# modin-project/modin

Measured on NVIDIA H100. Metric: rows/sec elementwise map (a*b+c) on 5e8x8 f64, higher is better.
Workload: dtype f64

## Files before the change

### modin_b200/csrc/elementwise.cu

```cuda
#include <type_traits>

#include "common.cuh"

namespace mb200 {

constexpr int kThreads = 256;
constexpr int kPair = 2;
constexpr int kSlab = kThreads * kPair;
constexpr int kSlabs = 8;
constexpr int kTile = kSlab * kSlabs;

struct MapParams {
  const void* in0[MB200_MAX_COLS];
  const void* in1[MB200_MAX_COLS];
  const void* in2[MB200_MAX_COLS];
  void* out[MB200_MAX_COLS];
  uint64_t s0[MB200_MAX_COLS];
  uint64_t s1[MB200_MAX_COLS];
  long long nrows;
};

template <typename T>
__device__ __forceinline__ T from_bits(uint64_t b);
template <>
__device__ __forceinline__ double from_bits<double>(uint64_t b) {
  return __longlong_as_double((long long)b);
}
template <>
__device__ __forceinline__ long long from_bits<long long>(uint64_t b) {
  return (long long)b;
}
template <>
__device__ __forceinline__ uint8_t from_bits<uint8_t>(uint64_t b) {
  return (uint8_t)(b != 0);
}

constexpr __host__ __device__ int op_nin(int op) { return op >= 64 ? 3 : (op >= 32 ? 2 : 1); }
constexpr __host__ __device__ bool op_is_pred(int op) {
  return op == MB200_OP_ISNA || op == MB200_OP_NOTNA || (op >= MB200_OP_EQ_S && op <= MB200_OP_GE_S) ||
         (op >= MB200_OP_EQ && op <= MB200_OP_GE);
}

template <int OP, typename TI, typename TO>
__device__ __forceinline__ TO apply(TI a, TI b, TI c, TI s0, TI s1) {
  constexpr bool F = std::is_same<TI, double>::value;
  if constexpr (OP == MB200_OP_ABS) {
    if constexpr (F) return (TO)fabs(a);
    else return (TO)(a < 0 ? (TI)(0ULL - (unsigned long long)a) : a);
  } else if constexpr (OP == MB200_OP_NEG) {
    if constexpr (F) return (TO)__longlong_as_double(__double_as_longlong(a) ^ (long long)0x8000000000000000ULL);
    else return (TO)(TI)(0ULL - (unsigned long long)a);
  } else if constexpr (OP == MB200_OP_ISNA) {
    return (TO)(a != a);
  } else if constexpr (OP == MB200_OP_NOTNA) {
    return (TO)(a == a);
  } else if constexpr (OP == MB200_OP_FILLNA_S) {
    return (TO)((a != a) ? s0 : a);
  } else if constexpr (OP == MB200_OP_AFFINE) {
    if constexpr (F) return (TO)__dadd_rn(__dmul_rn(a, s0), s1);
    else return (TO)(TI)((unsigned long long)a * (unsigned long long)s0 + (unsigned long long)s1);
  } else if constexpr (OP == MB200_OP_ADD_S || OP == MB200_OP_ADD) {
    TI r = (OP == MB200_OP_ADD) ? b : s0;
    if constexpr (F) return (TO)__dadd_rn(a, r);
    else return (TO)(TI)((unsigned long long)a + (unsigned long long)r);
  } else if constexpr (OP == MB200_OP_SUB_S || OP == MB200_OP_SUB) {
    TI r = (OP == MB200_OP_SUB) ? b : s0;
    if constexpr (F) return (TO)__dsub_rn(a, r);
    else return (TO)(TI)((unsigned long long)a - (unsigned long long)r);
  } else if constexpr (OP == MB200_OP_RSUB_S) {
    if constexpr (F) return (TO)__dsub_rn(s0, a);
    else return (TO)(TI)((unsigned long long)s0 - (unsigned long long)a);
  } else if constexpr (OP == MB200_OP_MUL_S || OP == MB200_OP_MUL) {
    TI r = (OP == MB200_OP_MUL) ? b : s0;
// ... 49 lines not shown
    return (TO)((a != a) ? b : a);
  } else if constexpr (OP == MB200_OP_FMA3) {
    if constexpr (F) return (TO)__dadd_rn(__dmul_rn(a, b), c);
    else return (TO)(TI)((unsigned long long)a * (unsigned long long)b + (unsigned long long)c);
  } else {
    return (TO)a;
  }
}

template <typename T>
struct Pair;
template <>
struct Pair<double> {
  using type = double2;
  static __device__ __forceinline__ double2 load(const double* p) { return ldg_stream_f64x2(p); }
  static __device__ __forceinline__ void store(double* p, const double2& v) { stg_stream_f64x2(p, v); }
};
template <>
struct Pair<long long> {
  using type = longlong2;
  static __device__ __forceinline__ longlong2 load(const long long* p) { return ldg_stream_i64x2(p); }
  static __device__ __forceinline__ void store(long long* p, const longlong2& v) { stg_stream_i64x2(p, v); }
};
template <>
struct Pair<uint8_t> {
  using type = uchar2;
  static __device__ __forceinline__ uchar2 load(const uint8_t* p) { return __ldg(reinterpret_cast<const uchar2*>(p)); }
  static __device__ __forceinline__ void store(uint8_t* p, const uchar2& v) { *reinterpret_cast<uchar2*>(p) = v; }
};

template <int OP, typename TI, typename TO, bool VEC>
__global__ void __launch_bounds__(kThreads) map_kernel(const __grid_constant__ MapParams p) {
  constexpr int NIN = op_nin(OP);
  const int tid = threadIdx.x;
  const int col = blockIdx.y;
  const long long base = (long long)blockIdx.x * kTile;
  const TI* __restrict__ a = static_cast<const TI*>(p.in0[col]);
  const TI* __restrict__ b = NIN >= 2 ? static_cast<const TI*>(p.in1[col]) : nullptr;
  const TI* __restrict__ c = NIN >= 3 ? static_cast<const TI*>(p.in2[col]) : nullptr;
  TO* __restrict__ o = static_cast<TO*>(p.out[col]);
  const TI s0 = from_bits<TI>(p.s0[col]);
  const TI s1 = from_bits<TI>(p.s1[col]);
  if (VEC && base + kTile <= p.nrows) {
    typename Pair<TI>::type va[kSlabs], vb[kSlabs], vc[kSlabs];
#pragma unroll
    for (int k = 0; k < kSlabs; ++k) {
      const long long i = base + k * kSlab + kPair * tid;
      va[k] = Pair<TI>::load(a + i);
      if constexpr (NIN >= 2) vb[k] = Pair<TI>::load(b + i);
      if constexpr (NIN >= 3) vc[k] = Pair<TI>::load(c + i);
    }
#pragma unroll
    for (int k = 0; k < kSlabs; ++k) {
      const long long i = base + k * kSlab + kPair * tid;
      TI bx = 0, by = 0, cx = 0, cy = 0;
      if constexpr (NIN >= 2) bx = vb[k].x, by = vb[k].y;
      if constexpr (NIN >= 3) cx = vc[k].x, cy = vc[k].y;
      typename Pair<TO>::type r;
      r.x = apply<OP, TI, TO>(va[k].x, bx, cx, s0, s1);
      r.y = apply<OP, TI, TO>(va[k].y, by, cy, s0, s1);
      Pair<TO>::store(o + i, r);
    }
  } else {
    const long long end = (base + kTile < p.nrows) ? base + kTile : p.nrows;
    for (long long i = base + tid; i < end; i += kThreads) {
      TI x = a[i];
      TI y = NIN >= 2 ? b[i] : (TI)0;
      TI z = NIN >= 3 ? c[i] : (TI)0;
      o[i] = apply<OP, TI, TO>(x, y, z, s0, s1);
    }
  }
}

#define MB_CASE(OPC, TI, TO)                                     \
  case OPC:                                                      \
    if (vec)                                                     \
      map_kernel<OPC, TI, TO, true><<<grid, kThreads, 0, st>>>(p);  \
    else                                                         \
      map_kernel<OPC, TI, TO, false><<<grid, kThreads, 0, st>>>(p); \
    MB_LAUNCH_CHECK("map_kernel");                               \
    return 0;

}

using namespace mb200;

extern "C" int mb200_map(int op, int dtype, int ncols, const void* const* in0, const void* const* in1,
                         const void* const* in2, void* const* out, int64_t nrows, const uint64_t* s0,
                         const uint64_t* s1, mb200_stream_t stream) {
  if (ncols < 0 || ncols > MB200_MAX_COLS) return fail("mb200_map", "ncols out of range (0..32)");
  if (nrows < 0) return fail("mb200_map", "negative nrows");
  if (ncols == 0 || nrows == 0) return 0;
  if (!in0 || !out) return fail("mb200_map", "null column array");
  const int nin = op_nin(op);
  if (nin >= 2 && !in1) return fail("mb200_map", "binary op needs in1");
  if (nin >= 3 && !in2) return fail("mb200_map", "ternary op needs in2");
  MapParams p;
  memset(&p, 0, sizeof(p));
  bool vec = true;
  for (int c = 0; c < ncols; ++c) {
    p.in0[c] = in0[c];
    p.in1[c] = nin >= 2 ? in1[c] : nullptr;
    p.in2[c] = nin >= 3 ? in2[c] : nullptr;
    p.out[c] = out[c];
    p.s0[c] = s0 ? s0[c] : 0;
    p.s1[c] = s1 ? s1[c] : 0;
    if (!in0[c] || !out[c]) return fail("mb200_map", "null column pointer");
    vec = vec && aligned16(in0[c]) && aligned16(out[c]);
    if (nin >= 2) vec = vec && in1[c] && aligned16(in1[c]);
    if (nin >= 3) vec = vec && in2[c] && aligned16(in2[c]);
    if ((nin >= 2 && !in1[c]) || (nin >= 3 && !in2[c])) return fail("mb200_map", "null column pointer");
  }
  p.nrows = nrows;
  const long long tiles_per_col = (nrows + kTile - 1) / kTile;
  if (tiles_per_col > 0x7fffffffLL) return fail("mb200_map", "too many rows for one launch");
  const dim3 grid((unsigned)tiles_per_col, (unsigned)ncols);
  cudaStream_t st = (cudaStream_t)stream;

  if (dtype == MB200_F64) {
    switch (op) {
      MB_CASE(MB200_OP_ABS, double, double)
      MB_CASE(MB200_OP_NEG, double, double)
      MB_CASE(MB200_OP_ISNA, double, uint8_t)
      MB_CASE(MB200_OP_NOTNA, double, uint8_t)
      MB_CASE(MB200_OP_FILLNA_S, double, double)
      MB_CASE(MB200_OP_AFFINE, double, double)
      MB_CASE(MB200_OP_ADD_S, double, double)
      MB_CASE(MB200_OP_SUB_S, double, double)
      MB_CASE(MB200_OP_RSUB_S, double, double)
      MB_CASE(MB200_OP_MUL_S, double, double)
      MB_CASE(MB200_OP_DIV_S, double, double)
      MB_CASE(MB200_OP_RDIV_S, double, double)
      MB_CASE(MB200_OP_EQ_S, double, uint8_t)
      MB_CASE(MB200_OP_NE_S, double, uint8_t)
      MB_CASE(MB200_OP_LT_S, double, uint8_t)
      MB_CASE(MB200_OP_LE_S, double, uint8_t)
      MB_CASE(MB200_OP_GT_S, double, uint8_t)
      MB_CASE(MB200_OP_GE_S, double, uint8_t)
      MB_CASE(MB200_OP_CLIP_S, double, double)
      MB_CASE(MB200_OP_COPY, double, double)
      MB_CASE(MB200_OP_ROUND_S, double, double)
      MB_CASE(MB200_OP_ORDERED_S, double, long long)
      MB_CASE(MB200_OP_ADD, double, double)
      MB_CASE(MB200_OP_SUB, double, double)
      MB_CASE(MB200_OP_MUL, double, double)
      MB_CASE(MB200_OP_DIV, double, double)
      MB_CASE(MB200_OP_EQ, double, uint8_t)
      MB_CASE(MB200_OP_NE, double, uint8_t)
      MB_CASE(MB200_OP_LT, double, uint8_t)
// ... 57 lines not shown
```

### modin_b200/csrc/groupby.cu

```cuda
#include "common.cuh"

namespace mb200 {

int sort_pairs_device(long long* keys, long long* pay, long long* tmp_keys, long long* tmp_pay,
                      unsigned int* counts, long long n, unsigned long long bias, int nbits, cudaStream_t st);
size_t sort_scratch_bytes(long long n);

struct __align__(16) Slot {
  long long key;
  int gid;
  int pad;
};

struct GbMeta {
  int ngroups;
  int overflow;
  long long kmin;
  long long kmax;
};

}

struct mb200_gb_table {
  mb200::Slot* slots;
  long long cap;
  double* acc;
  long long* cnt;
  long long* size;
  long long gcap;
  int nvals;
  int vstride;
  int flags;
  mb200::GbMeta* meta;
  int dense;
  long long kbase;
  unsigned int* present;
  long long nwords;
  unsigned int* blockoff;
  int borrowed;
  int skewed;
  int persisted;
  size_t carve_bytes, window_bytes;
  long long win_lo, win_hi;
  void* arena;
  size_t arena_bytes;
};

namespace mb200 {

constexpr int kGbThreads = 256;
constexpr int kGbWarps = kGbThreads / 32;
constexpr int kColStride = 34;
constexpr int kTileRows = 256;
constexpr int kTileColStride = 258;
constexpr int kGbStages = 3;
constexpr int kGbTmaThreads = kGbThreads + 32;
constexpr int kStageBytes = ((9 * kTileColStride * 8 + 127) / 128) * 128;

struct GbParams {
  Slot* slots;
  unsigned int mask;
  long long cap;
  double* acc;
  long long* cnt;
  long long* size;
  long long gcap;
  int nvals;
  int vstride;
  int flags;
  GbMeta* meta;
  const long long* keys;
  const void* vals[MB200_MAX_COLS];
  const void* pcnt[MB200_MAX_COLS];
  const long long* psize;
  long long nrows;
  int dense;
  long long kbase;
  unsigned int* present;
  int policy_mode;
  int prefetch;
};

__device__ __forceinline__ void red_add_f64(double* p, double v, uint64_t pol) {
  if (pol)
    asm volatile("red.relaxed.gpu.global.add.L2::cache_hint.f64 [%0], %1, %2;" ::"l"(p), "d"(v), "l"(pol) : "memory");
  else
    asm volatile("red.relaxed.gpu.global.add.f64 [%0], %1;" ::"l"(p), "d"(v) : "memory");
}
__device__ __forceinline__ void red_add_u64(long long* p, long long v, uint64_t) {
  asm volatile("red.relaxed.gpu.global.add.u64 [%0], %1;" ::"l"(p), "l"(v) : "memory");
// ... 234 lines not shown
            if (p.flags & MB200_GB_COUNT) {
              if (PARTIAL) red_add_u64(p.cnt + o, static_cast<const long long*>(p.pcnt[c0 + c])[base + r], keep);
              else if (xv == xv) red_add_u64(p.cnt + o, 1LL, keep);
            }
          }
        }
        if (p.dense && !(p.flags & MB200_GB_SIZE)) {
          seen |= __shfl_xor_sync(0xffffffffu, seen, 1);
          seen |= __shfl_xor_sync(0xffffffffu, seen, 2);
          seen |= __shfl_xor_sync(0xffffffffu, seen, 4);
          const unsigned int unseen = ~seen & rowok;
          if (c == 0 && unseen) {
#pragma unroll
            for (int kk = 0; kk < 8; ++kk)
              if ((unseen >> kk) & 1u) dense_mark(p, gs[kk]);
          }
        }
        __syncwarp();
      }
    }
  }
}

constexpr int kHotSlots = 256;
constexpr int kHotStride = 9;
constexpr int kHotStages = 2;
__host__ __device__ constexpr int hot_offset(int stages) {
  return ((stages * kStageBytes + 2 * stages * 8 + 63) / 64) * 64;
}
constexpr int kHotBytesSum = kHotSlots * 4 + kHotSlots * kHotStride * 8;
constexpr int kHotBytes = kHotBytesSum + kHotSlots * kHotStride * 4;
constexpr int kHotBit = 1 << 30;

template <bool HOT, int STAGES>
__global__ void __launch_bounds__(kGbTmaThreads) gb_accumulate_tma_kernel(const __grid_constant__ GbParams p,
                                                                          long long ntiles) {
  extern __shared__ __align__(128) unsigned char smem_raw[];
  uint64_t* full = reinterpret_cast<uint64_t*>(smem_raw + STAGES * kStageBytes);
  uint64_t* empty = full + STAGES;
  int* s_tag = reinterpret_cast<int*>(smem_raw + hot_offset(STAGES));
  double* s_hot = reinterpret_cast<double*>(smem_raw + hot_offset(STAGES) + kHotSlots * 4);
  unsigned int* s_hcnt = reinterpret_cast<unsigned int*>(smem_raw + hot_offset(STAGES) + kHotSlots * 4 + kHotSlots * kHotStride * 8);
  const int tid = threadIdx.x, lane = tid & 31, warp = tid >> 5;
  const int nv = p.nvals;
  const int gcap = (int)p.gcap;
  const long long first = blockIdx.x;
  const long long nmine = first < ntiles ? (ntiles - first + gridDim.x - 1) / gridDim.x : 0;

  if (HOT) {
    for (int i = tid; i < kHotSlots; i += kGbTmaThreads) s_tag[i] = -1;
    for (int i = tid; i < kHotSlots * kHotStride; i += kGbTmaThreads) {
      s_hot[i] = 0.0;
      if (p.flags & MB200_GB_COUNT) s_hcnt[i] = 0u;
    }
  }
  if (tid == 0) {
#pragma unroll
    for (int s = 0; s < STAGES; ++s) {
      mbar_init(&full[s], 1);
      mbar_init(&empty[s], kGbWarps);
    }
    mbar_fence_init();
  }
  __syncthreads();

  if (warp == kGbWarps) {
    if (lane == 0) {
      const uint64_t pol = l2_policy_evict_first();
      for (long long k = 0; k < nmine; ++k) {
        const int s = (int)(k % STAGES);
        if (k >= STAGES) mbar_wait(&empty[s], (uint32_t)(((k / STAGES) - 1) & 1));
        const long long row0 = (first + k * gridDim.x) * kTileRows;
        double* stage = reinterpret_cast<double*>(smem_raw + (size_t)s * kStageBytes);
        mbar_expect_tx(&full[s], (uint32_t)((1 + nv) * kTileRows * 8));
        tma_bulk_g2s(stage, p.keys + row0, kTileRows * 8, &full[s], pol);
        for (int c = 0; c < nv; ++c)
          tma_bulk_g2s(stage + (size_t)(1 + c) * kTileColStride, static_cast<const double*>(p.vals[c]) + row0,
                       kTileRows * 8, &full[s], pol);
      }
    }
    return;
  }
  const uint64_t keep = table_policy(p.policy_mode);
  const int c = lane & 7;
  for (long long k = 0; k < nmine; ++k) {
    const int s = (int)(k % STAGES);
    mbar_wait(&full[s], (uint32_t)((k / STAGES) & 1));
    const double* stage = reinterpret_cast<const double*>(smem_raw + (size_t)s * kStageBytes);
    const long long key = reinterpret_cast<const long long*>(stage)[warp * 32 + lane];
    if (p.prefetch && k + 1 < nmine) {
      const int s1 = (int)((k + 1) % STAGES);
      mbar_wait(&full[s1], (uint32_t)(((k + 1) / STAGES) & 1));
      const long long nk =
          reinterpret_cast<const long long*>(smem_raw + (size_t)s1 * kStageBytes)[warp * 32 + lane];
      const Slot* ns = &p.slots[hash_key(nk) & p.mask];
      asm volatile("prefetch.global.L2 [%0];" ::"l"(ns));
    }
    int gid = resolve_gid(p, key, keep);
    if ((p.flags & MB200_GB_SIZE) && gid < gcap) red_add_u64(p.size + gid, 1LL, keep);
    if (HOT && gid < gcap) {
      const int slot = gid & (kHotSlots - 1);
      int tag = *reinterpret_cast<volatile int*>(&s_tag[slot]);
      if (tag == -1) {
        const int old = atomicCAS(&s_tag[slot], -1, gid);
        tag = old == -1 ? gid : old;
      }
      if (tag == gid) gid |= kHotBit;
    }
    const double* vt = stage + kTileColStride + warp * 32;
    unsigned int seen = 0;
    int gs[8];
#pragma unroll
    for (int kk = 0; kk < 8; ++kk) {
      const int r = 4 * kk + (lane >> 3);
      const int pg = __shfl_sync(0xffffffffu, gid, r);
      const int g = HOT ? (pg & ~kHotBit) : pg;
      gs[kk] = g;
      if (c < nv && g < gcap) {
        const double xv = vt[c * kTileColStride + r];
        if (dense_visible(p, xv)) seen |= 1u << kk;
        if (xv == xv) {
          if (HOT && (pg & kHotBit)) {
            const int o = (g & (kHotSlots - 1)) * kHotStride + c;
            if (p.flags & MB200_GB_SUM) atomicAdd(&s_hot[o], xv);
            if (p.flags & MB200_GB_COUNT) atomicAdd(&s_hcnt[o], 1u);
          } else {
            const size_t o = (size_t)g * p.vstride + c;
            acc_update(p, o, xv, keep);
            if (p.flags & MB200_GB_COUNT) red_add_u64(p.cnt + o, 1LL, keep);
          }
        }
      }
    }
    if (p.dense && !(p.flags & MB200_GB_SIZE)) {
      seen |= __shfl_xor_sync(0xffffffffu, seen, 1);
      seen |= __shfl_xor_sync(0xffffffffu, seen, 2);
      seen |= __shfl_xor_sync(0xffffffffu, seen, 4);
      unsigned int unseen = ~seen & 0xffu;
      if (c == 0 && unseen) {
#pragma unroll
        for (int kk = 0; kk < 8; ++kk)
          if (((unseen >> kk) & 1u) && gs[kk] < gcap) dense_mark(p, gs[kk]);
      }
    }
    __syncwarp();
    if (lane == 0) mbar_arrive(&empty[s]);
  }
  if (HOT) {
    asm volatile("bar.sync 1, %0;" ::"n"(kGbThreads) : "memory");
    for (int i = tid; i < kHotSlots * 8; i += kGbThreads) {
      const int slot = i >> 3, cc = i & 7;
      const int tag = s_tag[slot];
      if (tag < 0 || cc >= nv) continue;
      const size_t o = (size_t)tag * p.vstride + cc;
      if (p.flags & MB200_GB_SUM) red_add_f64(p.acc + o, s_hot[slot * kHotStride + cc], 0);
      if ((p.flags & MB200_GB_COUNT) && s_hcnt[slot * kHotStride + cc])
        red_add_u64(p.cnt + o, (long long)s_hcnt[slot * kHotStride + cc], 0);
    }
  }
}

constexpr int kSmemThreads = 1024;

struct SmemTableLayout {
  unsigned int acc_off, cnt_off, size_off, present_off, total;
  int svs;
  int nrep;
  int rstride;
  int zstride;
};

__global__ void __launch_bounds__(kSmemThreads, 1) gb_accumulate_smem_kernel(const __grid_constant__ GbParams p,
                                                                             const SmemTableLayout lay) {
  extern __shared__ __align__(16) unsigned char smem_raw[];
// ... 68 lines not shown
      for (int r = 1; r < nrep; ++r) a += s_acc[r * rstride + o];
      red_add_f64(p.acc + i, a, 0);
    } else if (f_min || f_max) {
      long long a = s_acc_i[o];
      for (int r = 1; r < nrep; ++r) {
        const long long b = s_acc_i[r * rstride + o];
        a = f_min ? (b < a ? b : a) : (b > a ? b : a);
      }
      if (f_min && a != 0x7fffffffffffffffLL) red_min_s64(reinterpret_cast<long long*>(p.acc) + i, a);
      if (f_max && a != (long long)0x8000000000000000ULL) red_max_s64(reinterpret_cast<long long*>(p.acc) + i, a);
    }
    if (f_cnt) {
      long long n = 0;
      for (int r = 0; r < nrep; ++r) n += s_cnt[r * rstride + o];
      if (n) red_add_u64(p.cnt + i, n, 0);
    }
  }
  for (int g = tid; g < R; g += kSmemThreads) {
    if (!s_present[g]) continue;
    reinterpret_cast<unsigned char*>(p.present)[g] = 1;
    if (f_size) {
      long long n = 0;
      for (int r = 0; r < nrep; ++r) n += s_size[r * zstride + g];
      red_add_u64(p.size + g, n, 0);
    }
  }
}

__global__ void gb_fill_kernel(long long* p, long long n, long long v) {
  const long long stride = (long long)gridDim.x * blockDim.x;
  for (long long i = (long long)blockIdx.x * blockDim.x + threadIdx.x; i < n; i += stride) p[i] = v;
}

__global__ void gb_init_kernel(Slot* slots, long long cap, GbMeta* meta) {
  const long long i = (long long)blockIdx.x * blockDim.x + threadIdx.x;
  if (i < cap) {
    Slot s;
    s.key = 0;
    s.gid = -1;
    s.pad = 0;
    slots[i] = s;
  }
  if (i == 0) {
    meta->ngroups = 0;
    meta->overflow = 0;
    meta->kmin = 0x7fffffffffffffffLL;
    meta->kmax = (long long)0x8000000000000000ULL;
  }
}

__global__ void __launch_bounds__(256) gb_collect_kernel(const Slot* __restrict__ slots, long long cap, long long gcap,
                                                         long long* __restrict__ keys_by_gid,
                                                         long long* __restrict__ perm, GbMeta* meta) {
  __shared__ long long s_min[8], s_max[8];
  const long long i = (long long)blockIdx.x * blockDim.x + threadIdx.x;
  long long lo = 0x7fffffffffffffffLL, hi = (long long)0x8000000000000000ULL;
  if (i < cap) {
    const Slot s = slots[i];
    if (s.gid >= 0 && s.gid < gcap) {
      keys_by_gid[s.gid] = s.key;
      perm[s.gid] = s.gid;
      lo = hi = s.key;
    }
  }
#pragma unroll
  for (int m = 16; m >= 1; m >>= 1) {
// ... 172 lines not shown
    const unsigned int v = __shfl_up_sync(0xffffffffu, incl, m);
    if (lane >= m) incl += v;
  }
  if (lane == 31) s[warp] = incl;
  __syncthreads();
  unsigned int base = blockoff[blockIdx.x];
  for (int i = 0; i < warp; ++i) base += s[i];
  long long o = (long long)base + incl - c;
  while (bits) {
    const int b = __ffs(bits) - 1;
    bits &= bits - 1;
    const long long g = gid0 + w * 4 + (b >> 3);
    if (o < nout) {
      keys_out[o] = kbase + g;
      perm_out[o] = g;
    }
    ++o;
  }
}

static long long next_pow2(long long v) {
  long long p = 1;
  while (p < v) p <<= 1;
  return p;
}

static int gb_variant_from_env(size_t table_bytes, size_t l2_bytes) {
  const char* e = getenv("MB200_GB_VARIANT");
  if (e && e[0] == '0') return 0;
  if (e && e[0] == '1') return 1;
  if (e && e[0] == '2') return 2;
  (void)table_bytes;
  (void)l2_bytes;
  return 0;
}

template <int VARIANT, bool PARTIAL>
static int launch_ldg(const GbParams& p, const DevProps& dp, cudaStream_t st) {
  int occ = 0;
  MB_CUDA(cudaOccupancyMaxActiveBlocksPerMultiprocessor(&occ, gb_accumulate_kernel<VARIANT, PARTIAL>, kGbThreads, 0));
  const long long nchunks = (p.nrows + 31) / 32;
  long long grid = (long long)dp.sm_count * (occ < 1 ? 1 : occ);
  const long long need = (nchunks + kGbWarps - 1) / kGbWarps;
  if (grid > need) grid = need;
  gb_accumulate_kernel<VARIANT, PARTIAL><<<(unsigned)grid, kGbThreads, 0, st>>>(p);
  MB_LAUNCH_CHECK("gb_accumulate_kernel");
  return 0;
}

static int gb_launch(mb200_gb_table* t, const long long* keys, const void* const* vals, const void* const* pcnt,
                     const long long* psize, long long nrows, bool partial, cudaStream_t st) {
  if (nrows == 0) return 0;
  DevProps dp;
  if (int rc = dev_props(&dp)) return rc;
  GbParams p;
  memset(&p, 0, sizeof(p));
  p.slots = t->slots;
  p.mask = (unsigned int)(t->cap - 1);
  p.cap = t->cap;
  p.acc = t->acc;
  p.cnt = t->cnt;
  p.size = t->size;
  p.gcap = t->gcap;
  p.nvals = t->nvals;
  p.vstride = t->vstride;
  p.flags = t->flags;
// ... 6 lines not shown
  for (int c = 0; c < t->nvals; ++c) {
    p.vals[c] = vals ? vals[c] : nullptr;
    p.pcnt[c] = pcnt ? pcnt[c] : nullptr;
    if ((t->flags & (MB200_GB_SUM | MB200_GB_COUNT | MB200_GB_MIN | MB200_GB_MAX)) && !p.vals[c])
      return fail("groupby", "null value column");
    if (partial && (t->flags & MB200_GB_COUNT) && !p.pcnt[c]) return fail("groupby", "null partial count column");
    aligned = aligned && aligned16(p.vals[c]);
  }
  p.psize = psize;
  if (partial && (t->flags & MB200_GB_SIZE) && !psize) return fail("groupby", "null partial size column");
  p.nrows = nrows;
  {
    const char* e = getenv("MB200_GB_POLICY");
    p.policy_mode = (e && e[0] == 'l') ? 1 : ((e && e[0] == 'n' && e[1] == 'o' && e[2] == 'r') ? 2 : ((e && e[0] == 'u') ? 3 : 0));
    const char* pf = getenv("MB200_GB_PREFETCH");
    p.prefetch = (pf && pf[0] == '1') ? 1 : 0;
  }
  const size_t table_bytes = (size_t)t->cap * sizeof(Slot) + (size_t)t->gcap * t->vstride * 8 *
                                                                  (((t->flags & (MB200_GB_SUM | MB200_GB_MIN | MB200_GB_MAX)) ? 1 : 0) +
                                                                   ((t->flags & MB200_GB_COUNT) ? 1 : 0));
  const int variant = gb_variant_from_env(table_bytes, dp.l2_bytes);

  struct WindowGuard {
    cudaStream_t st;
    bool on = false;
    ~WindowGuard() {
      if (on) {
        cudaStreamAttrValue v;
        memset(&v, 0, sizeof(v));
        cudaStreamSetAttribute(st, cudaStreamAttributeAccessPolicyWindow, &v);
      }
    }
  } guard{st};
  {
    const char* e = getenv("MB200_GB_PERSIST");
    const size_t acc_bytes = (size_t)t->gcap * t->vstride * 8;
    const bool off = e && e[0] == '0';
    void* win_base = t->dense ? (void*)t->acc : t->arena;
    const size_t win_bytes = t->dense ? acc_bytes : t->arena_bytes;
    const bool want = !off && win_base && win_bytes >= ((size_t)8 << 20);
    if (want) {
      if (!t->persisted) {
        size_t mw = 0;
        const size_t mp = l2_carveout_acquire(&mw);
        if (mp) {
          t->persisted = 1;
          t->carve_bytes = mp;
          t->window_bytes = mw;
        }
      }
      if (t->persisted) {
        cudaStreamAttrValue v;
        memset(&v, 0, sizeof(v));
        v.accessPolicyWindow.base_ptr = win_base;
        v.accessPolicyWindow.num_bytes = win_bytes < t->window_bytes ? win_bytes : t->window_bytes;
        const double fit = (double)t->carve_bytes / (double)v.accessPolicyWindow.num_bytes;
        v.accessPolicyWindow.hitRatio = fit >= 1.0 ? 1.0f : (float)fit;
        v.accessPolicyWindow.hitProp = cudaAccessPropertyPersisting;
        v.accessPolicyWindow.missProp = cudaAccessPropertyNormal;
        if (cudaStreamSetAttribute(st, cudaStreamAttributeAccessPolicyWindow, &v) == cudaSuccess) guard.on = true;
        else cudaGetLastError();
      }
    }
  }

  if (t->dense && !partial) {
    const char* e = getenv("MB200_GB_SMEM");
    SmemTableLayout lay;
    lay.svs = t->vstride + 1;
    lay.rstride = (int)((((size_t)t->gcap * lay.svs + 15) & ~(size_t)15) + 1);
    lay.zstride = (int)(t->gcap | 1);
    size_t off = 0;
    for (int nrep = 32; nrep >= 1; nrep >>= 1) {
      const size_t elems = (size_t)nrep * lay.rstride;
      off = 0;
      lay.nrep = nrep;
      lay.acc_off = (unsigned)off;
      if (t->flags & (MB200_GB_SUM | MB200_GB_MIN | MB200_GB_MAX)) off += elems * 8;
      lay.cnt_off = (unsigned)off;
      if (t->flags & MB200_GB_COUNT) off += (elems * 4 + 15) & ~(size_t)15;
      lay.size_off = (unsigned)off;
      if (t->flags & MB200_GB_SIZE) off += (((size_t)nrep * lay.zstride * 4) + 15) & ~(size_t)15;
      lay.present_off = (unsigned)off;
      off += ((size_t)t->gcap + 15) & ~(size_t)15;
      lay.total = (unsigned)off;
      if (off <= dp.smem_optin) break;
    }
    if (!(e && e[0] == '0') && off <= dp.smem_optin) {
      MB_CUDA(cudaFuncSetAttribute(gb_accumulate_smem_kernel, cudaFuncAttributeMaxDynamicSharedMemorySize, (int)off));
      long long grid = dp.sm_count;
      const long long need = (nrows + kSmemThreads - 1) / kSmemThreads;
      if (grid > need) grid = need;
      gb_accumulate_smem_kernel<<<(unsigned)grid, kSmemThreads, off, st>>>(p, lay);
      MB_LAUNCH_CHECK("gb_accumulate_smem_kernel");
      return 0;
    }
  }
  if (variant == 0 && !partial && aligned && t->nvals <= 8 && nrows >= kTileRows) {
    const long long ntiles = nrows / kTileRows;
    const bool hot = t->skewed && !(t->flags & (MB200_GB_MIN | MB200_GB_MAX | MB200_GB_SIZE));
    const char* se = getenv("MB200_GB_STAGES");
    const bool two = !hot && !t->dense && !(se && se[0] == '3');
    const size_t smem = hot   ? (size_t)hot_offset(kHotStages) + ((t->flags & MB200_GB_COUNT) ? kHotBytes : kHotBytesSum)
                        : two ? (size_t)2 * kStageBytes + 2 * 2 * sizeof(uint64_t)
                              : (size_t)kGbStages * kStageBytes + 2 * kGbStages * sizeof(uint64_t);
    auto kern = hot   ? gb_accumulate_tma_kernel<true, kHotStages>
                : two ? gb_accumulate_tma_kernel<false, 2>
                      : gb_accumulate_tma_kernel<false, kGbStages>;
    MB_CUDA(cudaFuncSetAttribute(kern, cudaFuncAttributeMaxDynamicSharedMemorySize, (int)smem));
    int occ = 0;
    MB_CUDA(cudaOccupancyMaxActiveBlocksPerMultiprocessor(&occ, kern, kGbTmaThreads, smem));
    long long grid = (long long)dp.sm_count * (occ < 1 ? 1 : occ);
    if (grid > ntiles) grid = ntiles;
    kern<<<(unsigned)grid, kGbTmaThreads, smem, st>>>(p, ntiles);
    MB_LAUNCH_CHECK("gb_accumulate_tma_kernel");
    const long long done = ntiles * kTileRows;
    if (done == nrows) return 0;
    p.keys = keys + done;
    for (int c = 0; c < t->nvals; ++c)
      if (p.vals[c]) p.vals[c] = static_cast<const double*>(p.vals[c]) + done;
    p.nrows = nrows - done;
  }
  if (variant == 2) {
    if (partial) return launch_ldg<1, true>(p, dp, st);
    return launch_ldg<1, false>(p, dp, st);
  }
  if (partial) return launch_ldg<0, true>(p, dp, st);
  return launch_ldg<0, false>(p, dp, st);
}

}

using namespace mb200;

struct DenseArrays {
  void* acc;
  void* cnt;
  void* size;
  void* present;
};

static int gb_create_impl(mb200_gb_table** table, int64_t group_capacity, int nvals, int flags, bool dense,
                          int64_t kbase, const DenseArrays& ext, mb200_stream_t stream, bool init_arrays = true);

extern "C" int mb200_gb_create(mb200_gb_table** table, int64_t group_capacity, int nvals, int flags,
                               mb200_stream_t stream) {
  return gb_create_impl(table, group_capacity, nvals, flags, false, 0, DenseArrays{}, stream);
}
// ... 162 lines not shown
  }
  if ((flags & MB200_GB_COUNT) && init_arrays) {
    if (!t->borrowed && dense) MB_TRY(cudaMallocAsync((void**)&t->cnt, accb, st));
    MB_TRY(cudaMemsetAsync(t->cnt, 0, accb, st));
  }
  if ((flags & MB200_GB_SIZE) && init_arrays) {
    if (!t->borrowed && dense) MB_TRY(cudaMallocAsync((void**)&t->size, (size_t)t->gcap * 8, st));
    MB_TRY(cudaMemsetAsync(t->size, 0, (size_t)t->gcap * 8, st));
  }
#undef MB_TRY
  gb_init_kernel<<<(unsigned)(dense ? 1 : (t->cap + 255) / 256), 256, 0, st>>>(t->slots, t->cap, t->meta);
  e = cudaGetLastError();
  if (e != cudaSuccess) goto bad;
  g_launches.fetch_add(1);
  *table = t;
  return 0;
bad:
  mb200_gb_destroy(t, stream);
  return cuda_fail("mb200_gb_create", e);
}

extern "C" int mb200_gb_destroy(mb200_gb_table* t, mb200_stream_t stream) {
  if (!t) return 0;
  cudaStream_t st = (cudaStream_t)stream;
  if (t->arena) cudaFreeAsync(t->arena, st);
  if (t->meta) cudaFreeAsync(t->meta, st);
  if (!t->borrowed && !t->arena) {
    if (t->acc) cudaFreeAsync(t->acc, st);
    if (t->cnt) cudaFreeAsync(t->cnt, st);
    if (t->size) cudaFreeAsync(t->size, st);
    if (t->present) cudaFreeAsync(t->present, st);
  }
  if (t->blockoff) cudaFreeAsync(t->blockoff, st);
  if (t->persisted) l2_carveout_release();
  delete t;
  return 0;
}

extern "C" int mb200_l2_persist_info(int* max_persist_bytes, int* max_window_bytes) {
  int dev = 0;
  MB_CUDA(cudaGetDevice(&dev));
  if (max_persist_bytes) MB_CUDA(cudaDeviceGetAttribute(max_persist_bytes, cudaDevAttrMaxPersistingL2CacheSize, dev));
  if (max_window_bytes) MB_CUDA(cudaDeviceGetAttribute(max_window_bytes, cudaDevAttrMaxAccessPolicyWindowSize, dev));
  return 0;
}

extern "C" int mb200_gb_accumulate(mb200_gb_table* t, const int64_t* keys, const void* const* vals,
                                   int64_t nrows, mb200_stream_t stream) {
  if (!t) return fail("mb200_gb_accumulate", "null table");
  if (nrows < 0) return fail("mb200_gb_accumulate", "negative nrows");
  if (nrows > 0 && !keys) return fail("mb200_gb_accumulate", "null keys");
  return gb_launch(t, reinterpret_cast<const long long*>(keys), vals, nullptr, nullptr, nrows, false,
                   (cudaStream_t)stream);
}

extern "C" int mb200_gb_merge_partial(mb200_gb_table* t, const int64_t* keys, const void* const* sums,
                                      const void* const* cnts, const int64_t* sizes, int64_t npartial,
                                      mb200_stream_t stream) {
  if (!t) return fail("mb200_gb_merge_partial", "null table");
  if (npartial < 0) return fail("mb200_gb_merge_partial", "negative npartial");
  if (npartial > 0 && !keys) return fail("mb200_gb_merge_partial", "null keys");
  return gb_launch(t, reinterpret_cast<const long long*>(keys), sums, cnts, reinterpret_cast<const long long*>(sizes),
                   npartial, true, (cudaStream_t)stream);
}

static int dense_finalize_presence(mb200_gb_table* t, cudaStream_t st) {
// ... 137 lines not shown
```

Before: 22.99 billion.

## Enlarge affine map tiles and add column-slab groupby passes sized to L2

The elementwise map kernel now picks its tile depth per op: f64 AFFINE uses 32 slabs per block instead of 8, so each thread keeps more loads in flight and fewer blocks are launched. The grid is computed per case to match. Separately, groupby gains a multi-pass mode for dense tables that processes a few value columns at a time into an L2-sized scratch slab and then folds the partial results back. This trades extra passes and fold kernels for better L2 residency. The larger map tile raises register use per thread, which may lower occupancy.

```diff
diff --git a/modin_b200/csrc/elementwise.cu b/modin_b200/csrc/elementwise.cu
--- a/modin_b200/csrc/elementwise.cu
+++ b/modin_b200/csrc/elementwise.cu
@@ -7,8 +7,7 @@
 constexpr int kThreads = 256;
 constexpr int kPair = 2;
 constexpr int kSlab = kThreads * kPair;
-constexpr int kSlabs = 8;
-constexpr int kTile = kSlab * kSlabs;
+
 
 struct MapParams {
   const void* in0[MB200_MAX_COLS];
@@ -39,6 +38,11 @@
 constexpr __host__ __device__ bool op_is_pred(int op) {
   return op == MB200_OP_ISNA || op == MB200_OP_NOTNA || (op >= MB200_OP_EQ_S && op <= MB200_OP_GE_S) ||
          (op >= MB200_OP_EQ && op <= MB200_OP_GE);
+}
+
+template <int OP, typename TI, typename TO>
+constexpr __host__ __device__ int map_slabs() {
+  return (OP == MB200_OP_AFFINE && sizeof(TI) == 8) ? 32 : 8;
 }
 
 template <int OP, typename TI, typename TO>
@@ -154,6 +158,8 @@
 template <int OP, typename TI, typename TO, bool VEC>
 __global__ void __launch_bounds__(kThreads) map_kernel(const __grid_constant__ MapParams p) {
   constexpr int NIN = op_nin(OP);
+  constexpr int kSlabs = map_slabs<OP, TI, TO>();
+  constexpr int kTile = kSlab * kSlabs;
   const int tid = threadIdx.x;
   const int col = blockIdx.y;
   const long long base = (long long)blockIdx.x * kTile;
@@ -196,6 +202,7 @@
 
 #define MB_CASE(OPC, TI, TO)                                     \
   case OPC:                                                      \
+    grid.x = (unsigned)((nrows + kSlab * map_slabs<OPC, TI, TO>() - 1) / (kSlab * map_slabs<OPC, TI, TO>())); \
     if (vec)                                                     \
       map_kernel<OPC, TI, TO, true><<<grid, kThreads, 0, st>>>(p);  \
     else                                                         \
@@ -234,9 +241,9 @@
     if ((nin >= 2 && !in1[c]) || (nin >= 3 && !in2[c])) return fail("mb200_map", "null column pointer");
   }
   p.nrows = nrows;
-  const long long tiles_per_col = (nrows + kTile - 1) / kTile;
+  const long long tiles_per_col = (nrows + kSlab * 8 - 1) / (kSlab * 8);
   if (tiles_per_col > 0x7fffffffLL) return fail("mb200_map", "too many rows for one launch");
-  const dim3 grid((unsigned)tiles_per_col, (unsigned)ncols);
+  dim3 grid(1u, (unsigned)ncols);
   cudaStream_t st = (cudaStream_t)stream;
 
   if (dtype == MB200_F64) {
diff --git a/modin_b200/csrc/groupby.cu b/modin_b200/csrc/groupby.cu
--- a/modin_b200/csrc/groupby.cu
+++ b/modin_b200/csrc/groupby.cu
@@ -44,6 +44,8 @@
   long long win_lo, win_hi;
   void* arena;
   size_t arena_bytes;
+  void* slab;
+  size_t slab_bytes;
 };
 
 namespace mb200 {
@@ -52,10 +54,13 @@
 constexpr int kGbWarps = kGbThreads / 32;
 constexpr int kColStride = 34;
 constexpr int kTileRows = 256;
-constexpr int kTileColStride = 258;
+__host__ __device__ constexpr int tile_col_stride(int lanes) { return kTileRows + 16 / lanes; }
 constexpr int kGbStages = 3;
 constexpr int kGbTmaThreads = kGbThreads + 32;
-constexpr int kStageBytes = ((9 * kTileColStride * 8 + 127) / 128) * 128;
+__host__ __device__ constexpr int tma_stage_bytes(int lanes) {
+  return (((1 + lanes) * tile_col_stride(lanes) * 8 + 127) / 128) * 128;
+}
+constexpr int kStageBytes = tma_stage_bytes(8);
 
 struct GbParams {
   Slot* slots;
@@ -356,11 +361,16 @@
 constexpr int kHotBytes = kHotBytesSum + kHotSlots * kHotStride * 4;
 constexpr int kHotBit = 1 << 30;
 
-template <bool HOT, int STAGES>
+template <bool HOT, int STAGES, int LANES = 8>
 __global__ void __launch_bounds__(kGbTmaThreads) gb_accumulate_tma_kernel(const __grid_constant__ GbParams p,
                                                                           long long ntiles) {
+  static_assert(LANES == 8 || LANES == 4 || LANES == 2 || LANES == 1, "lanes per row");
+  static_assert(!HOT || LANES == 8, "the hot-group cache is 8 columns wide");
+  constexpr int kStage = tma_stage_bytes(LANES);
+  constexpr int kCol = tile_col_stride(LANES);
+  constexpr int kRowsPerStep = 32 / LANES;
   extern __shared__ __align__(128) unsigned char smem_raw[];
-  uint64_t* full = reinterpret_cast<uint64_t*>(smem_raw + STAGES * kStageBytes);
+  uint64_t* full = reinterpret_cast<uint64_t*>(smem_raw + STAGES * kStage);
   uint64_t* empty = full + STAGES;
   int* s_tag = reinterpret_cast<int*>(smem_raw + hot_offset(STAGES));
   double* s_hot = reinterpret_cast<double*>(smem_raw + hot_offset(STAGES) + kHotSlots * 4);
@@ -395,28 +405,28 @@
         const int s = (int)(k % STAGES);
         if (k >= STAGES) mbar_wait(&empty[s], (uint32_t)(((k / STAGES) - 1) & 1));
         const long long row0 = (first + k * gridDim.x) * kTileRows;
-        double* stage = reinterpret_cast<double*>(smem_raw + (size_t)s * kStageBytes);
+        double* stage = reinterpret_cast<double*>(smem_raw + (size_t)s * kStage);
         mbar_expect_tx(&full[s], (uint32_t)((1 + nv) * kTileRows * 8));
         tma_bulk_g2s(stage, p.keys + row0, kTileRows * 8, &full[s], pol);
         for (int c = 0; c < nv; ++c)
-          tma_bulk_g2s(stage + (size_t)(1 + c) * kTileColStride, static_cast<const double*>(p.vals[c]) + row0,
+          tma_bulk_g2s(stage + (size_t)(1 + c) * kCol, static_cast<const double*>(p.vals[c]) + row0,
                        kTileRows * 8, &full[s], pol);
       }
     }
     return;
   }
   const uint64_t keep = table_policy(p.policy_mode);
-  const int c = lane & 7;
+  const int c = lane & (LANES - 1);
   for (long long k = 0; k < nmine; ++k) {
     const int s = (int)(k % STAGES);
     mbar_wait(&full[s], (uint32_t)((k / STAGES) & 1));
-    const double* stage = reinterpret_cast<const double*>(smem_raw + (size_t)s * kStageBytes);
+    const double* stage = reinterpret_cast<const double*>(smem_raw + (size_t)s * kStage);
     const long long key = reinterpret_cast<const long long*>(stage)[warp * 32 + lane];
     if (p.prefetch && k + 1 < nmine) {
       const int s1 = (int)((k + 1) % STAGES);
       mbar_wait(&full[s1], (uint32_t)(((k + 1) / STAGES) & 1));
       const long long nk =
-          reinterpret_cast<const long long*>(smem_raw + (size_t)s1 * kStageBytes)[warp * 32 + lane];
+          reinterpret_cast<const long long*>(smem_raw + (size_t)s1 * kStage)[warp * 32 + lane];
       const Slot* ns = &p.slots[hash_key(nk) & p.mask];
       asm volatile("prefetch.global.L2 [%0];" ::"l"(ns));
     }
@@ -431,17 +441,17 @@
       }
       if (tag == gid) gid |= kHotBit;
     }
-    const double* vt = stage + kTileColStride + warp * 32;
+    const double* vt = stage + kCol + warp * 32;
     unsigned int seen = 0;
-    int gs[8];
-#pragma unroll
-    for (int kk = 0; kk < 8; ++kk) {
-      const int r = 4 * kk + (lane >> 3);
+    int gs[LANES];
+#pragma unroll
+    for (int kk = 0; kk < LANES; ++kk) {
+      const int r = kRowsPerStep * kk + lane / LANES;
       const int pg = __shfl_sync(0xffffffffu, gid, r);
       const int g = HOT ? (pg & ~kHotBit) : pg;
       gs[kk] = g;
       if (c < nv && g < gcap) {
-        const double xv = vt[c * kTileColStride + r];
+        const double xv = vt[c * kCol + r];
         if (dense_visible(p, xv)) seen |= 1u << kk;
         if (xv == xv) {
           if (HOT && (pg & kHotBit)) {
@@ -457,13 +467,12 @@
       }
     }
     if (p.dense && !(p.flags & MB200_GB_SIZE)) {
-      seen |= __shfl_xor_sync(0xffffffffu, seen, 1);
-      seen |= __shfl_xor_sync(0xffffffffu, seen, 2);
-      seen |= __shfl_xor_sync(0xffffffffu, seen, 4);
-      unsigned int unseen = ~seen & 0xffu;
+#pragma unroll
+      for (int m = 1; m < LANES; m <<= 1) seen |= __shfl_xor_sync(0xffffffffu, seen, m);
+      unsigned int unseen = ~seen & ((1u << LANES) - 1u);
       if (c == 0 && unseen) {
 #pragma unroll
-        for (int kk = 0; kk < 8; ++kk)
+        for (int kk = 0; kk < LANES; ++kk)
           if (((unseen >> kk) & 1u) && gs[kk] < gcap) dense_mark(p, gs[kk]);
       }
     }
@@ -598,6 +607,30 @@
   for (long long i = (long long)blockIdx.x * blockDim.x + threadIdx.x; i < n; i += stride) p[i] = v;
 }
 
+__global__ void __launch_bounds__(256) gb_slab_fold_kernel(long long* __restrict__ acc, long long* __restrict__ cnt,
+                                                           const long long* __restrict__ sacc,
+                                                           const long long* __restrict__ scnt, long long R, int lw,
+                                                           int nv, int vstride, int c0, int flags) {
+  const long long n = R << lw;
+  const long long stride = (long long)gridDim.x * blockDim.x;
+  for (long long i = (long long)blockIdx.x * blockDim.x + threadIdx.x; i < n; i += stride) {
+    const long long g = i >> lw;
+    const int c = (int)(i & ((1 << lw) - 1));
+    if (c >= nv) continue;
+    const size_t o = (size_t)g * vstride + c0 + c;
+    if (sacc) {
+      const long long v = sacc[i];
+      if (flags & MB200_GB_SUM) {
+        reinterpret_cast<double*>(acc)[o] += __longlong_as_double(v);
+      } else {
+        const long long a = acc[o];
+        acc[o] = (flags & MB200_GB_MIN) ? (v < a ? v : a) : (v > a ? v : a);
+      }
+    }
+    if (scnt) cnt[o] += scnt[i];
+  }
+}
+
 __global__ void gb_init_kernel(Slot* slots, long long cap, GbMeta* meta) {
   const long long i = (long long)blockIdx.x * blockDim.x + threadIdx.x;
   if (i < cap) {
@@ -836,6 +869,69 @@
   if (e && e[0] == '2') return 2;
   (void)table_bytes;
   (void)l2_bytes;
+  return 0;
+}
+
+constexpr double kSlabL2Share = 0.625;
+static int slab_width(long long R, int narrays, size_t budget) {
+  for (int w = 8; w >= 1; w >>= 1)
+    if ((size_t)R * w * 8 * narrays <= budget) return w;
+  return 8;
+}
+
+template <typename Kernel>
+static int launch_tma(Kernel kern, size_t smem, const GbParams& p, long long ntiles, const DevProps& dp,
+                      cudaStream_t st) {
+  MB_CUDA(cudaFuncSetAttribute(kern, cudaFuncAttributeMaxDynamicSharedMemorySize, (int)smem));
+  int occ = 0;
+  MB_CUDA(cudaOccupancyMaxActiveBlocksPerMultiprocessor(&occ, kern, kGbTmaThreads, smem));
+  long long grid = (long long)dp.sm_count * (occ < 1 ? 1 : occ);
+  if (grid > ntiles) grid = ntiles;
+  kern<<<(unsigned)grid, kGbTmaThreads, smem, st>>>(p, ntiles);
+  MB_LAUNCH_CHECK("gb_accumulate_tma_kernel");
+  return 0;
+}
+
+template <int LANES>
+static int launch_tma_slab(const GbParams& q, long long ntiles, const DevProps& dp, cudaStream_t st) {
+  return launch_tma(gb_accumulate_tma_kernel<false, kGbStages, LANES>,
+                    (size_t)kGbStages * tma_stage_bytes(LANES) + 2 * kGbStages * sizeof(uint64_t), q, ntiles, dp, st);
+}
+
+static int slab_passes(const mb200_gb_table* t, const GbParams& p, int w, long long ntiles, const DevProps& dp,
+                       cudaStream_t st) {
+  const long long R = t->gcap;
+  const bool has_acc = t->flags & (MB200_GB_SUM | MB200_GB_MIN | MB200_GB_MAX);
+  long long* sacc = has_acc ? static_cast<long long*>(t->slab) : nullptr;
+  long long* scnt = (t->flags & MB200_GB_COUNT) ? static_cast<long long*>(t->slab) + (has_acc ? R * w : 0) : nullptr;
+  const long long ident = (t->flags & MB200_GB_MIN) ? 0x7fffffffffffffffLL : (long long)0x8000000000000000ULL;
+  const int lw = w == 4 ? 2 : (w == 2 ? 1 : 0);
+  long long fgrid = (R * w + 255) / 256;
+  if (fgrid > (long long)dp.sm_count * 16) fgrid = (long long)dp.sm_count * 16;
+  for (int c0 = 0; c0 < t->nvals; c0 += w) {
+    GbParams q = p;
+    q.acc = reinterpret_cast<double*>(sacc);
+    q.cnt = scnt;
+    q.vstride = w;
+    q.nvals = t->nvals - c0 < w ? t->nvals - c0 : w;
+    for (int c = 0; c < MB200_MAX_COLS; ++c) q.vals[c] = c < q.nvals ? p.vals[c0 + c] : nullptr;
+    if (c0 > 0) {
+      q.flags &= ~MB200_GB_SIZE;
+      q.size = nullptr;
+    }
+    if (sacc) {
+      gb_fill_kernel<<<(unsigned)fgrid, 256, 0, st>>>(sacc, R * w, ident);
+      MB_LAUNCH_CHECK("gb_fill_kernel");
+    }
+    if (scnt) MB_CUDA(cudaMemsetAsync(scnt, 0, (size_t)R * w * 8, st));
+    const int rc = w == 4   ? launch_tma_slab<4>(q, ntiles, dp, st)
+                   : w == 2 ? launch_tma_slab<2>(q, ntiles, dp, st)
+                            : launch_tma_slab<1>(q, ntiles, dp, st);
+    if (rc) return rc;
+    gb_slab_fold_kernel<<<(unsigned)fgrid, 256, 0, st>>>(reinterpret_cast<long long*>(t->acc), t->cnt, sacc, scnt, R,
+                                                         lw, q.nvals, t->vstride, c0, t->flags);
+    MB_LAUNCH_CHECK("gb_slab_fold_kernel");
+  }
   return 0;
 }
 
@@ -908,35 +1004,54 @@
       }
     }
   } guard{st};
+  const bool has_acc = t->flags & (MB200_GB_SUM | MB200_GB_MIN | MB200_GB_MAX);
+  const int narrays = (has_acc ? 1 : 0) + ((t->flags & MB200_GB_COUNT) ? 1 : 0);
+  const bool slab_ok = variant == 0 && t->dense && !partial && !t->skewed && aligned && t->nvals <= 8 &&
+                       nrows >= kTileRows && narrays > 0;
+  int slab_w = 8;
   {
     const char* e = getenv("MB200_GB_PERSIST");
     const size_t acc_bytes = (size_t)t->gcap * t->vstride * 8;
     const bool off = e && e[0] == '0';
     void* win_base = t->dense ? (void*)t->acc : t->arena;
-    const size_t win_bytes = t->dense ? acc_bytes : t->arena_bytes;
+    size_t win_bytes = t->dense ? acc_bytes : t->arena_bytes;
     const bool want = !off && win_base && win_bytes >= ((size_t)8 << 20);
-    if (want) {
-      if (!t->persisted) {
-        size_t mw = 0;
-        const size_t mp = l2_carveout_acquire(&mw);
-        if (mp) {
-          t->persisted = 1;
-          t->carve_bytes = mp;
-          t->window_bytes = mw;
+    if (want && !t->persisted) {
+      size_t mw = 0;
+      const size_t mp = l2_carveout_acquire(&mw);
+      if (mp) {
+        t->persisted = 1;
+        t->carve_bytes = mp;
+        t->window_bytes = mw;
+      }
+    }
+    const bool pin = want && t->persisted;
+    if (slab_ok) {
+      slab_w = slab_width(t->gcap, narrays, pin ? t->carve_bytes : (size_t)(kSlabL2Share * (double)dp.l2_bytes));
+      if (slab_w < t->nvals) {
+        const size_t need = (size_t)t->gcap * slab_w * 8 * narrays;
+        if (t->slab_bytes < need) {
+          if (t->slab) MB_CUDA(cudaFreeAsync(t->slab, st));
+          t->slab = nullptr;
+          t->slab_bytes = 0;
+          MB_CUDA(cudaMallocAsync(&t->slab, need, st));
+          t->slab_bytes = need;
         }
+        win_base = t->slab;
+        win_bytes = need;
       }
-      if (t->persisted) {
-        cudaStreamAttrValue v;
-        memset(&v, 0, sizeof(v));
-        v.accessPolicyWindow.base_ptr = win_base;
-        v.accessPolicyWindow.num_bytes = win_bytes < t->window_bytes ? win_bytes : t->window_bytes;
-        const double fit = (double)t->carve_bytes / (double)v.accessPolicyWindow.num_bytes;
-        v.accessPolicyWindow.hitRatio = fit >= 1.0 ? 1.0f : (float)fit;
-        v.accessPolicyWindow.hitProp = cudaAccessPropertyPersisting;
-        v.accessPolicyWindow.missProp = cudaAccessPropertyNormal;
-        if (cudaStreamSetAttribute(st, cudaStreamAttributeAccessPolicyWindow, &v) == cudaSuccess) guard.on = true;
-        else cudaGetLastError();
-      }
+    }
+    if (pin) {
+      cudaStreamAttrValue v;
+      memset(&v, 0, sizeof(v));
+      v.accessPolicyWindow.base_ptr = win_base;
+      v.accessPolicyWindow.num_bytes = win_bytes < t->window_bytes ? win_bytes : t->window_bytes;
+      const double fit = (double)t->carve_bytes / (double)v.accessPolicyWindow.num_bytes;
+      v.accessPolicyWindow.hitRatio = fit >= 1.0 ? 1.0f : (float)fit;
+      v.accessPolicyWindow.hitProp = cudaAccessPropertyPersisting;
+      v.accessPolicyWindow.missProp = cudaAccessPropertyNormal;
+      if (cudaStreamSetAttribute(st, cudaStreamAttributeAccessPolicyWindow, &v) == cudaSuccess) guard.on = true;
+      else cudaGetLastError();
     }
   }
 
@@ -977,19 +1092,17 @@
     const bool hot = t->skewed && !(t->flags & (MB200_GB_MIN | MB200_GB_MAX | MB200_GB_SIZE));
     const char* se = getenv("MB200_GB_STAGES");
     const bool two = !hot && !t->dense && !(se && se[0] == '3');
-    const size_t smem = hot   ? (size_t)hot_offset(kHotStages) + ((t->flags & MB200_GB_COUNT) ? kHotBytes : kHotBytesSum)
-                        : two ? (size_t)2 * kStageBytes + 2 * 2 * sizeof(uint64_t)
-                              : (size_t)kGbStages * kStageBytes + 2 * kGbStages * sizeof(uint64_t);
-    auto kern = hot   ? gb_accumulate_tma_kernel<true, kHotStages>
-                : two ? gb_accumulate_tma_kernel<false, 2>
-                      : gb_accumulate_tma_kernel<false, kGbStages>;
-    MB_CUDA(cudaFuncSetAttribute(kern, cudaFuncAttributeMaxDynamicSharedMemorySize, (int)smem));
-    int occ = 0;
-    MB_CUDA(cudaOccupancyMaxActiveBlocksPerMultiprocessor(&occ, kern, kGbTmaThreads, smem));
-    long long grid = (long long)dp.sm_count * (occ < 1 ? 1 : occ);
-    if (grid > ntiles) grid = ntiles;
-    kern<<<(unsigned)grid, kGbTmaThreads, smem, st>>>(p, ntiles);
-    MB_LAUNCH_CHECK("gb_accumulate_tma_kernel");
+    if (slab_w < t->nvals) {
+      if (int rc = slab_passes(t, p, slab_w, ntiles, dp, st)) return rc;
+    } else {
+      const size_t smem = hot   ? (size_t)hot_offset(kHotStages) + ((t->flags & MB200_GB_COUNT) ? kHotBytes : kHotBytesSum)
+                          : two ? (size_t)2 * kStageBytes + 2 * 2 * sizeof(uint64_t)
+                                : (size_t)kGbStages * kStageBytes + 2 * kGbStages * sizeof(uint64_t);
+      auto kern = hot   ? gb_accumulate_tma_kernel<true, kHotStages>
+                  : two ? gb_accumulate_tma_kernel<false, 2>
+                        : gb_accumulate_tma_kernel<false, kGbStages>;
+      if (int rc = launch_tma(kern, smem, p, ntiles, dp, st)) return rc;
+    }
     const long long done = ntiles * kTileRows;
     if (done == nrows) return 0;
     p.keys = keys + done;
@@ -1218,6 +1331,7 @@
     if (t->present) cudaFreeAsync(t->present, st);
   }
   if (t->blockoff) cudaFreeAsync(t->blockoff, st);
+  if (t->slab) cudaFreeAsync(t->slab, st);
   if (t->persisted) l2_carveout_release();
   delete t;
   return 0;
```

Result: no change. 23.03 billion (median of 6 runs) (+0.1%).
